# FocoosAI/focoos

Hardware: AMD Instinct MI355X
Metric: images/sec @ 640^2 (infer bs=32) (higher is better)
Workload: dtype bf16; 1 GPU; fai-detr-l-obj365 inference, bf16 MFMA, bs=32/GPU, 640x640, random-init weights (seed 0), uint8 HWC images resident in HBM, device post-process + D2H of packed detections included; global_batch=32, parallelism=replicas x1 (no data-path collective), steps_are=hipGraph replays, batches_in_flight=3, concurrent_batch_parts=1

## Files before the change

### focoos_amd/csrc/conv_pw_chain.hip

```cpp
#include "pw_common.h"

struct PwChainArgs {
  const bf16_t* x1;
  const bf16_t* x2;
  const bf16_t* res;
  const bf16_t* w1p;
  const bf16_t* w2p;
  const float* b1;
  const float* b2;
  bf16_t* y1;
  bf16_t* y2;
  int ldx1, ldx2, ldr, ldy1, ldy2;
  int M, N1, act1, act2;
  unsigned x1_bytes, x2_bytes, r_bytes;
  bf16_t* pool;
  int ldp, H, W;
};

template <int RL, typename F>
__device__ __forceinline__ void pw_dma_rows_map(__amdgpu_buffer_rsrc_t r, unsigned char* tile, int nrows, int ld, int col0, int wave, int lane, F&& pix) {
  const int ninstr = nrows * RL / 64;
  for (int i = wave; i < ninstr; i += 4) {
    const int q = i * 64 + lane;
    const int row = q / RL, pc = q % RL;
    const int lc = pw_swz<RL>(row, pc);
    const int m = pix(row);
    const unsigned off = (m >= 0) ? (unsigned)(m * ld + col0 + lc * 8) * 2u : FX_OOB;
    pw_dma16(r, tile + i * 1024, off);
  }
}

template <int K1A, int K1B, int N2, int BM, bool QUAD = false>
__global__ __launch_bounds__(256, ((N2 <= 64 && K1B == 0) ? 4 : ((N2 <= 128 && (K1B == 0 || N2 <= 64)) ? 3 : 2))) void pw_chain_kernel(const PwChainArgs p) {
  constexpr int K1 = K1A + K1B, KS1 = K1 / 16, KS1A = K1A / 16;
  constexpr int RLA = K1A / 8, RLB = (K1B > 0 ? K1B : 64) / 8;
  constexpr int TM = BM / 32;
  constexpr int XA_BYTES = BM * K1A * 2, XB_BYTES = BM * K1B * 2;
  constexpr int PF1 = KS1 < 4 ? KS1 : 4;
  constexpr bool HAS2 = N2 > 0;
  constexpr int WN2 = !HAS2 ? 1 : (N2 >= 128 ? 4 : 2), WM2 = 4 / WN2;
  constexpr int TN2 = !HAS2 ? 1 : N2 / (32 * WN2), TM2 = BM / (32 * WM2);
  constexpr int RL2 = (HAS2 ? N2 : 64) / 8;
  constexpr int PF2 = 4;
  static_assert(BM == 64, "64-pixel tiles");
  static_assert(K1A % 64 == 0 && K1B % 64 == 0 && PF1 == 4, "K segments in multiples of 64 (= whole blocks of 4 k-steps)");
  static_assert(!HAS2 || (N2 % 64 == 0 && N2 <= 256), "N2");
  extern __shared__ __attribute__((aligned(16))) unsigned char smem[];
  unsigned char* XA = smem;
  unsigned char* XB = smem + XA_BYTES;
  unsigned char* T = smem + XA_BYTES + XB_BYTES;

  const int tid = threadIdx.x, lane = tid & 63;
  const int wave = __builtin_amdgcn_readfirstlane(tid >> 6);
  const int l32 = lane & 31, half = lane >> 5;
  const int m0 = blockIdx.x * BM;
  const int NG = p.N1 >> 8;
  const int KS2 = p.N1 >> 4;

  __shared__ int s_pix[QUAD ? BM : 1];
  if constexpr (QUAD) {
    if (tid < BM) {
      const int W2 = p.W >> 1, QI = (p.H >> 1) * W2;
      const int q = blockIdx.x * (BM / 4) + (tid >> 2), sub = tid & 3;
      int m = -1;
      if (q * 4 < p.M) {
        const int b = q / QI, rem = q - b * QI;
        const int y2 = rem / W2, x2 = rem - y2 * W2;
        m = (b * p.H + 2 * y2 + (sub >> 1)) * p.W + 2 * x2 + (sub & 1);
      }
      s_pix[tid] = m;
    }
    __syncthreads();
  }
  auto pix = [&](int row) -> int {
    if constexpr (!QUAD) {
      const int m = m0 + row;
      return m < p.M ? m : -1;
    } else {
      return s_pix[row];
    }
  };
  const __amdgpu_buffer_rsrc_t x1r = __builtin_amdgcn_make_buffer_rsrc((void*)p.x1, 0, p.x1_bytes, 0x00020000);
  pw_dma_rows_map<RLA>(x1r, XA, BM, p.ldx1, 0, wave, lane, pix);
  if constexpr (K1B > 0) {
    const __amdgpu_buffer_rsrc_t x2r = __builtin_amdgcn_make_buffer_rsrc((void*)p.x2, 0, p.x2_bytes, 0x00020000);
    pw_dma_rows_map<RLB>(x2r, XB, BM, p.ldx2, 0, wave, lane, pix);
  }
  const __amdgpu_buffer_rsrc_t rr = __builtin_amdgcn_make_buffer_rsrc((void*)(p.res ? p.res : p.x1), 0, p.res ? p.r_bytes : 0u, 0x00020000);

  const int wn2 = wave % WN2, wm2 = wave / WN2;
  f32x16 acc2[TN2][TM2];
#pragma unroll
  for (int a = 0; a < TN2; ++a)
#pragma unroll
    for (int b = 0; b < TM2; ++b)
#pragma unroll
      for (int r = 0; r < 16; ++r) acc2[a][b][r] = 0.0f;

  for (int g = 0; g < NG; ++g) {
    int l32g = l32, halfg = half, tidg = tid;
    asm volatile("" : "+v"(l32g), "+v"(halfg), "+v"(tidg));
    if (p.res) pw_dma_rows_map<32>(rr, T, BM, p.ldr, g * 256, wave, lane, pix);
    bf16x8 a2[PF2][TN2];
    const bf16_t* w2 = p.w2p + (size_t)((wn2 * TN2) * KS2 + g * 16) * 512 + lane * 8;
    if constexpr (HAS2) {
#pragma unroll
      for (int i = 0; i < PF2; ++i)
#pragma unroll
        for (int a = 0; a < TN2; ++a) a2[i][a] = pw_ldg_frag(w2 + (size_t)(a * KS2 + i) * 512);
    }
#pragma unroll
    for (int a = 0; a < 2; ++a) {
      const bf16_t* w1 = p.w1p + (size_t)((g * 8 + wave * 2 + a) * KS1) * 512 + lane * 8;
      bf16x8 a1[PF1];
#pragma unroll
      for (int i = 0; i < PF1; ++i) a1[i] = pw_ldg_frag(w1 + i * 512);
      f32x16 acc[TM];
#pragma unroll
      for (int gq = 0; gq < 4; ++gq) {
        const float4 bb = *reinterpret_cast<const float4*>(p.b1 + g * 256 + wave * 64 + a * 32 + 8 * gq + 4 * halfg);
#pragma unroll
        for (int b = 0; b < TM; ++b) {
          acc[b][4 * gq] = bb.x; acc[b][4 * gq + 1] = bb.y; acc[b][4 * gq + 2] = bb.z; acc[b][4 * gq + 3] = bb.w;
        }
      }
      if (a == 0) {
        asm volatile("s_waitcnt vmcnt(0)" ::: "memory");
        __syncthreads();
      }
#define FX_PW_STEPS(XT_, KROW_, RL_, KL0_)                                                                                  \
  _Pragma("unroll") for (int i = 0; i < PF1; ++i) {                                                                         \
    bf16x8 xb[TM];                                                                                                          \
    _Pragma("unroll") for (int b = 0; b < TM; ++b) {                                                                        \
      const int row = b * 32 + l32k;                                                                                         \
      xb[b] = *reinterpret_cast<const bf16x8*>((XT_) + row * ((KROW_)*2) + (pw_swz<RL_>(row, ((KL0_) + i) * 2 + halfg) << 4)); \
    }                                                                                                                       \
    _Pragma("unroll") for (int b = 0; b < TM; ++b) acc[b] = FX_MFMA_32x32x16(a1[i], xb[b], acc[b]); \
    const int kn = ks0 + i + PF1;                                                                                           \
    a1[i] = pw_ldg_frag(w1 + (kn < KS1 ? kn : KS1 - 1) * 512);  \
  }
#pragma unroll 1
      for (int ks0 = 0; ks0 < KS1; ks0 += PF1) {
        int l32k = l32g;
        asm volatile("" : "+v"(l32k));
        if (K1B == 0 || ks0 < KS1A) {
          FX_PW_STEPS(XA, K1A, RLA, ks0)
        } else {
          FX_PW_STEPS(XB, (K1B > 0 ? K1B : 64), RLB, ks0 - KS1A)
        }
      }
#undef FX_PW_STEPS
#pragma unroll
      for (int b = 0; b < TM; ++b)
#pragma unroll
        for (int gq = 0; gq < 4; ++gq) {
          const int row = b * 32 + l32g;
          const int chunk = wave * 8 + a * 4 + gq;
          unsigned char* tp = T + row * 512 + ((chunk ^ (row & 15)) << 4) + halfg * 8;
          float v0 = acc[b][4 * gq], v1 = acc[b][4 * gq + 1], v2 = acc[b][4 * gq + 2], v3 = acc[b][4 * gq + 3];
          if (p.res) {
            const uint2 r2 = *reinterpret_cast<const uint2*>(tp);
            v0 += bf16lo_to_f32(r2.x);
            v1 += bf16hi_to_f32(r2.x);
            v2 += bf16lo_to_f32(r2.y);
            v3 += bf16hi_to_f32(r2.y);
          }
          if (p.act1 == FX_ACT_RELU) {
            v0 = fmaxf(v0, 0.0f); v1 = fmaxf(v1, 0.0f); v2 = fmaxf(v2, 0.0f); v3 = fmaxf(v3, 0.0f);
          }
          uint2 o;
          o.x = pack_bf16x2(v0, v1);
          o.y = pack_bf16x2(v2, v3);
          *reinterpret_cast<uint2*>(tp) = o;
        }
    }
    __syncthreads();
#pragma unroll
    for (int i = 0; i < BM * 32 / 256; ++i) {
      const int q = tidg + i * 256;
      const int row = q >> 5, lc = q & 31;
      const uint4 v = *reinterpret_cast<const uint4*>(T + row * 512 + ((lc ^ (row & 15)) << 4));
      const int m = pix(row);
      if (m >= 0 && p.y1) *reinterpret_cast<uint4*>(p.y1 + (size_t)m * p.ldy1 + g * 256 + lc * 8) = v;
    }
    if constexpr (QUAD) {
#pragma unroll
      for (int i = 0; i < (BM / 4) * 32 / 256; ++i) {
        const int idx = tidg + i * 256;
        const int j = idx >> 5, lc = idx & 31;
        float s8[8] = {0, 0, 0, 0, 0, 0, 0, 0};
#pragma unroll
        for (int r = 0; r < 4; ++r) {
          const int row = 4 * j + r;
          float f[8];
          unpack_bf16x8(*reinterpret_cast<const uint4*>(T + row * 512 + ((lc ^ (row & 15)) << 4)), f);
#pragma unroll
          for (int e = 0; e < 8; ++e) s8[e] += f[e];
        }
#pragma unroll
        for (int e = 0; e < 8; ++e) s8[e] *= 0.25f;
        const int q = blockIdx.x * (BM / 4) + j;
        if (q * 4 < p.M) *reinterpret_cast<uint4*>(p.pool + (size_t)q * p.ldp + g * 256 + lc * 8) = pack_bf16x8(s8);
      }
    }
    if constexpr (HAS2) {
#pragma unroll
      for (int ks = 0; ks < 16; ++ks) {
        bf16x8 tb[TM2];
#pragma unroll
        for (int b = 0; b < TM2; ++b) {
          const int row = (wm2 * TM2 + b) * 32 + l32g;
          tb[b] = *reinterpret_cast<const bf16x8*>(T + row * 512 + (((ks * 2 + halfg) ^ (row & 15)) << 4));
        }
#pragma unroll
        for (int a = 0; a < TN2; ++a)
#pragma unroll
          for (int b = 0; b < TM2; ++b) acc2[a][b] = FX_MFMA_32x32x16(a2[ks % PF2][a], tb[b], acc2[a][b]);
        if (ks + PF2 < 16) {
#pragma unroll
          for (int a = 0; a < TN2; ++a) a2[ks % PF2][a] = pw_ldg_frag(w2 + (size_t)(a * KS2 + ks + PF2) * 512);
        }
      }
    }
    __syncthreads();
  }

  if constexpr (HAS2) {
#pragma unroll
    for (int a = 0; a < TN2; ++a)
#pragma unroll
      for (int gq = 0; gq < 4; ++gq) {
        const int n = (wn2 * TN2 + a) * 32 + 8 * gq + 4 * half;
        const float4 bb = *reinterpret_cast<const float4*>(p.b2 + n);
#pragma unroll
        for (int b = 0; b < TM2; ++b) {
          const int row = (wm2 * TM2 + b) * 32 + l32;
          float v0 = acc2[a][b][4 * gq] + bb.x, v1 = acc2[a][b][4 * gq + 1] + bb.y;
          float v2 = acc2[a][b][4 * gq + 2] + bb.z, v3 = acc2[a][b][4 * gq + 3] + bb.w;
          if (p.act2 == FX_ACT_RELU) {
            v0 = fmaxf(v0, 0.0f); v1 = fmaxf(v1, 0.0f); v2 = fmaxf(v2, 0.0f); v3 = fmaxf(v3, 0.0f);
          }
          uint2 o;
          o.x = pack_bf16x2(v0, v1);
          o.y = pack_bf16x2(v2, v3);
          *reinterpret_cast<uint2*>(T + row * (N2 * 2) + (pw_swz<RL2>(row, n >> 3) << 4) + half * 8) = o;
        }
      }
    __syncthreads();
#pragma unroll
    for (int i = 0; i < BM * RL2 / 256; ++i) {
      const int q = tid + i * 256;
      const int row = q / RL2, lc = q % RL2;
      const uint4 v = *reinterpret_cast<const uint4*>(T + row * (N2 * 2) + (pw_swz<RL2>(row, lc) << 4));
      const int m = pix(row);
      if (m >= 0) *reinterpret_cast<uint4*>(p.y2 + (size_t)m * p.ldy2 + lc * 8) = v;
    }
  }
}

template <int K1A, int K1B, int N2, bool QUAD = false>
static int launch_pw_chain(const PwChainArgs& a, hipStream_t stream) {
  constexpr int BM = 64;
  constexpr int SMEM = BM * (K1A + K1B) * 2 + BM * 512;
  static bool attr_set = false;
  auto kern = pw_chain_kernel<K1A, K1B, N2, BM, QUAD>;
  if (!attr_set) {
    if (hipFuncSetAttribute(reinterpret_cast<const void*>(kern), hipFuncAttributeMaxDynamicSharedMemorySize, SMEM) != hipSuccess)
      return FX_ERR_RUNTIME;
    attr_set = true;
  }
  hipLaunchKernelGGL(kern, dim3((a.M + BM - 1) / BM), dim3(256), SMEM, stream, a);
  return fx_launch_status();
}

#define FX_PW_INSTANCES(X)                                                                             \
  X(64, 0, 0) X(64, 0, 64) X(64, 0, 128) X(64, 64, 0) X(64, 64, 64) X(64, 64, 128)                     \
  X(128, 0, 0) X(128, 0, 128) X(128, 0, 256) X(128, 256, 0) X(128, 256, 128) X(128, 256, 256)          \
  X(256, 0, 0) X(256, 0, 256) X(256, 512, 0) X(256, 512, 256)

extern "C" int fx_pw_chain_supported(int K1a, int K1b, int N1, int N2) {
  if (N1 <= 0 || N1 % 256 != 0) return 0;
#define FX_PW_CASE(KA, KB, NN2) \
  if (K1a == KA && K1b == KB && N2 == NN2) return 1;
  FX_PW_INSTANCES(FX_PW_CASE)
#undef FX_PW_CASE
  return 0;
}

#define FX_PW_POOL_INSTANCES(X) X(64, 0, 128) X(128, 0, 256)

extern "C" int fx_pw_chain_pool_supported(int K1a, int K1b, int N1, int N2) {
  if (N1 <= 0 || N1 % 256 != 0) return 0;
#define FX_PW_CASE(KA, KB, NN2) \
  if (K1a == KA && K1b == KB && N2 == NN2) return 1;
  FX_PW_POOL_INSTANCES(FX_PW_CASE)
#undef FX_PW_CASE
  return 0;
}

extern "C" int fx_pw_chain_bf16(const fx_pw_chain_desc* d, fx_stream_t stream_) {
  FX_CHECK_ARG(d && d->x1 && d->w1 && d->bias1 && d->M > 0);
  FX_CHECK_ARG(d->y1 || (d->pool && d->N2 > 0));
  FX_CHECK_ARG(d->K1b == 0 || d->x2);
  FX_CHECK_ARG((d->act1 == FX_ACT_NONE || d->act1 == FX_ACT_RELU) && (d->act2 == FX_ACT_NONE || d->act2 == FX_ACT_RELU));
  FX_CHECK_ARG(d->N2 == 0 || (d->w2 && d->bias2 && d->y2));
  if (!fx_pw_chain_supported(d->K1a, d->K1b, d->N1, d->N2)) return FX_ERR_UNSUPPORTED;
  FX_CHECK_ARG(d->ldx1 >= d->K1a && d->ldx1 % 8 == 0 && (!d->y1 || (d->ldy1 >= d->N1 && d->ldy1 % 8 == 0)));
  FX_CHECK_ARG(d->K1b == 0 || (d->ldx2 >= d->K1b && d->ldx2 % 8 == 0));
  FX_CHECK_ARG(!d->residual || (d->ldr >= d->N1 && d->ldr % 8 == 0));
  FX_CHECK_ARG(d->N2 == 0 || (d->ldy2 >= d->N2 && d->ldy2 % 8 == 0));
  FX_CHECK_ARG(((uintptr_t)d->x1 % 16) == 0 && ((uintptr_t)d->x2 % 16) == 0 && ((uintptr_t)d->residual % 16) == 0);
  FX_CHECK_ARG(((uintptr_t)d->w1 % 16) == 0 && ((uintptr_t)d->w2 % 16) == 0 && ((uintptr_t)d->y1 % 16) == 0 && ((uintptr_t)d->y2 % 16) == 0);
  FX_CHECK_ARG(((uintptr_t)d->bias1 % 16) == 0 && ((uintptr_t)d->bias2 % 16) == 0);
  const int64_t x1_bytes = ((int64_t)d->M - 1) * d->ldx1 * 2 + (int64_t)d->K1a * 2;
  const int64_t x2_bytes = d->K1b ? ((int64_t)d->M - 1) * d->ldx2 * 2 + (int64_t)d->K1b * 2 : 0;
  const int64_t r_bytes = d->residual ? ((int64_t)d->M - 1) * d->ldr * 2 + (int64_t)d->N1 * 2 : 0;
  if (x1_bytes >= 0xFFFFFFF0ll || x2_bytes >= 0xFFFFFFF0ll || r_bytes >= 0xFFFFFFF0ll) return FX_ERR_UNSUPPORTED;
  PwChainArgs a;
  a.x1 = reinterpret_cast<const bf16_t*>(d->x1);
  a.x2 = reinterpret_cast<const bf16_t*>(d->x2);
  a.res = reinterpret_cast<const bf16_t*>(d->residual);
  a.w1p = reinterpret_cast<const bf16_t*>(d->w1);
  a.w2p = reinterpret_cast<const bf16_t*>(d->w2);
  a.b1 = d->bias1;
  a.b2 = d->bias2;
  a.y1 = reinterpret_cast<bf16_t*>(d->y1);
  a.y2 = reinterpret_cast<bf16_t*>(d->y2);
  a.ldx1 = d->ldx1; a.ldx2 = d->ldx2; a.ldr = d->ldr; a.ldy1 = d->ldy1; a.ldy2 = d->ldy2;
  a.M = d->M; a.N1 = d->N1; a.act1 = d->act1; a.act2 = d->act2;
  a.x1_bytes = (unsigned)x1_bytes; a.x2_bytes = (unsigned)x2_bytes; a.r_bytes = (unsigned)r_bytes;
  a.pool = reinterpret_cast<bf16_t*>(d->pool); a.ldp = d->ldp; a.H = d->img_h; a.W = d->img_w;
  hipStream_t stream = reinterpret_cast<hipStream_t>(stream_);
  if (d->pool) {
    FX_CHECK_ARG(d->img_h > 0 && d->img_w > 0 && d->img_h % 2 == 0 && d->img_w % 2 == 0 && d->M % (d->img_h * d->img_w) == 0);
    FX_CHECK_ARG(d->ldp >= d->N1 && d->ldp % 8 == 0 && ((uintptr_t)d->pool % 16) == 0);
    if (!fx_pw_chain_pool_supported(d->K1a, d->K1b, d->N1, d->N2)) return FX_ERR_UNSUPPORTED;
#define FX_PW_CASE(KA, KB, NN2) \
  if (d->K1a == KA && d->K1b == KB && d->N2 == NN2) return launch_pw_chain<KA, KB, NN2, true>(a, stream);
    FX_PW_POOL_INSTANCES(FX_PW_CASE)
#undef FX_PW_CASE
    return FX_ERR_UNSUPPORTED;
  }
#define FX_PW_CASE(KA, KB, NN2) \
  if (d->K1a == KA && d->K1b == KB && d->N2 == NN2) return launch_pw_chain<KA, KB, NN2>(a, stream);
  FX_PW_INSTANCES(FX_PW_CASE)
#undef FX_PW_CASE
  return FX_ERR_UNSUPPORTED;
}
```

### focoos_amd/csrc/conv_pw_kplane.hip

```cpp
#include <type_traits>

#include "pw_common.h"

#ifndef FX_PWK_RES_DEPTH
#define FX_PWK_RES_DEPTH 3
#endif

int fx_tune(const char* env_name, int default_value);

struct PWKArgs {
  const bf16_t* x;
  const bf16_t* wp;
  const float* bias;
  const bf16_t* res;
  bf16_t* y;
  int N, ldx, ldy, ldr, M;
  int ntg;
  int HW;
  int64_t y_bstride;
  unsigned x_bytes, r_bytes;
  int rot;
};

template <int OFF>
__device__ __forceinline__ void pwk_ldg(bf16x8& dst, unsigned voff, const bf16_t* sbase) {
  asm volatile("global_load_dwordx4 %0, %1, %2 offset:%3" : "+v"(dst) : "v"(voff), "s"(sbase), "n"(OFF) : "memory");
}
typedef __attribute__((address_space(3))) const bf16x8 pwk_lds_frag_t;
template <int IMM>
__device__ __forceinline__ bf16x8 pwk_lds_read(int addr) {
  return *reinterpret_cast<pwk_lds_frag_t*>((size_t)(unsigned)(addr + IMM));
}
__device__ __forceinline__ float pwk_act(float v, std::integral_constant<int, FX_ACT_RELU>) { return fmaxf(v, 0.0f); }
__device__ __forceinline__ float pwk_act(float v, std::integral_constant<int, FX_ACT_SILU>) { return v * __builtin_amdgcn_rcpf(1.0f + __expf(-v)); }
__device__ __forceinline__ float pwk_act(float v, std::integral_constant<int, FX_ACT_NONE>) { return v; }

template <int K, int ACT, int RESMODE, int TM = 4, int ABL = 0>
__global__ __launch_bounds__(256, TM == 4 ? 2 : 3) void conv_pw_kplane_kernel(const PWKArgs p) {
  constexpr int TN = 2, NW = 4, BM = TM * 32, BN = 256;
  constexpr int NTHR = 256, NDW = NTHR / 64;
  constexpr int KS = K / 16;
  constexpr int PLANE = BM * 16, XBYTES = 2 * KS * PLANE;
  constexpr int PF = 4;
  static_assert(KS % PF == 0 && (KS - 1) * PLANE < 65536, "plane offsets are 16-bit immediates");
  extern __shared__ __attribute__((aligned(16))) unsigned char smem[];
  float* biasL = reinterpret_cast<float*>(smem + XBYTES);

  const int tid = threadIdx.x, lane = tid & 63;
  const int wave = __builtin_amdgcn_readfirstlane(tid >> 6);
  const int l32 = lane & 31, half = lane >> 5;
  const int m0 = fx_xcd_remap(blockIdx.x, gridDim.x) * BM;
  const int nt_first = blockIdx.y * p.ntg;
  const int NT = min(p.N / BN, nt_first + p.ntg);
  const int cnt = NT - nt_first;
  const int rot = p.rot ? (int)(blockIdx.x % (unsigned)cnt) : 0;
  auto tile_of = [&](int k) { const int t = k + rot; return nt_first + (t >= cnt ? t - cnt : t); };

  for (int i = tid; i < p.N; i += NTHR) biasL[i] = p.bias ? p.bias[i] : 0.0f;
  {
    const __amdgpu_buffer_rsrc_t xr = __builtin_amdgcn_make_buffer_rsrc((void*)p.x, 0, p.x_bytes, 0x00020000);
    constexpr int NP = K / 8;
    static_assert(BM % 64 == 0, "64-row DMA blocks");
    for (int i = wave; i < (BM / 64) * NP; i += NDW) {
      const int blk = i / NP, c = i % NP;
      const int m = m0 + blk * 64 + lane;
      const int pln = (c & 1) * KS + (c >> 1);
      if constexpr (!(ABL & 16)) pw_dma16(xr, smem + pln * PLANE + blk * 1024, m < p.M ? (unsigned)(m * p.ldx + c * 8) * 2u : FX_OOB);
    }
  }
  f32x16 acc[TN][TM];
  bf16x8 ar[PF][TN];
  const unsigned wvoff = lane * 16;
  const bf16_t* wwave = p.wp + (size_t)(wave * TN) * KS * 512;
  auto w_ptr = [&](int a, int nt, int ks) -> const bf16_t* { return wwave + ((size_t)(nt * 8 + a) * KS + ks) * 512; };
#pragma unroll
  for (int a = 0; a < TN; ++a) {
    const bf16_t* w0 = w_ptr(a, tile_of(0), 0);
    c3_static_for<PF>([&](auto ic) {
      constexpr int i = decltype(ic)::value;
      ar[i][a] = bf16x8{0, 0, 0, 0, 0, 0, 0, 0};
      pwk_ldg<i * 1024>(ar[i][a], wvoff, w0);
    });
  }
  const int lds0 = (int)(unsigned)(size_t)((__attribute__((address_space(3))) unsigned char*)smem);
  int addr[TM];
#pragma unroll
  for (int b = 0; b < TM; ++b) addr[b] = lds0 + (b * 32 + l32) * 16 + half * KS * PLANE;
  asm volatile("s_waitcnt vmcnt(0)" ::: "memory");
  __syncthreads();

  for (int kt = 0; kt < cnt; ++kt) {
    const int nt = tile_of(kt);
    const int n0 = nt * BN;
    const int ntn = kt + 1 < cnt ? tile_of(kt + 1) : nt;
#pragma unroll
    for (int a = 0; a < TN; ++a)
#pragma unroll
      for (int gq = 0; gq < 4; ++gq) {
        const float4 bb = *reinterpret_cast<const float4*>(biasL + n0 + (wave * TN + a) * 32 + 8 * gq + 4 * half);
#pragma unroll
        for (int b = 0; b < TM; ++b) {
          acc[a][b][4 * gq] = bb.x; acc[a][b][4 * gq + 1] = bb.y; acc[a][b][4 * gq + 2] = bb.z; acc[a][b][4 * gq + 3] = bb.w;
        }
      }
    bf16x8 xb[2][TM];
#pragma unroll
    for (int b = 0; b < TM; ++b) xb[0][b] = pwk_lds_read<0>(addr[b]);
#pragma unroll 1
    for (int g = 0; g < KS / PF; ++g) {
      const bool last = g == KS / PF - 1;
      const bf16_t* wnext[TN];
#pragma unroll
      for (int a = 0; a < TN; ++a) wnext[a] = w_ptr(a, last ? ntn : nt, last ? 0 : (g + 1) * PF);
      const int aoff = g * PF * PLANE;
      auto kstep = [&](auto jc) {
        constexpr int j = decltype(jc)::value;
        if constexpr (TN == 1) c3_wait<(PF - 1) * TN>(ar[j][0]); else c3_wait<(PF - 1) * TN>(ar[j][0], ar[j][1]);
#pragma unroll
        for (int a = 0; a < TN; ++a) {
#pragma unroll
          for (int b = 0; b < TM; ++b) {
            if constexpr (!(ABL & 8)) acc[a][b] = FX_MFMA_32x32x16(ar[j][a], xb[j & 1][b], acc[a][b]);
            if (a == 0) {
              if constexpr (j + 1 < PF) xb[(j + 1) & 1][b] = pwk_lds_read<(j + 1) * PLANE>(addr[b] + aoff);
              else xb[0][b] = pwk_lds_read<PF * PLANE>(addr[b] + (last ? -PF * PLANE : aoff));
            }
            if constexpr (!(ABL & 1)) {
              if (b == TM - 1) pwk_ldg<j * 1024>(ar[j][a], wvoff, wnext[a]);
            }
            __builtin_amdgcn_sched_barrier(0);
          }
        }
      };
      c3_static_for<PF>(kstep);
    }
    constexpr int RD = (FX_PWK_RES_DEPTH < TM) ? FX_PWK_RES_DEPTH : TM;
    constexpr int RS = RD + 1 > TM ? TM : RD + 1;
    uint4 rr[RS][TN * 2];
    if constexpr (ABL & 4) {
#pragma unroll
      for (int i = 0; i < RS * TN * 2; ++i) (&rr[0][0])[i] = make_uint4(0, 0, 0, 0);
    }
    auto ld_res = [&](int b, uint4* dst) {
      const int m = min(m0 + b * 32 + l32, p.M - 1);
      const bf16_t* rrow = p.res + (size_t)m * p.ldr + n0 + wave * TN * 32 + half * 8;
#pragma unroll
      for (int a = 0; a < TN; ++a)
#pragma unroll
        for (int g2 = 0; g2 < 2; ++g2) dst[a * 2 + g2] = *reinterpret_cast<const uint4*>(rrow + a * 32 + g2 * 16);
    };
    if constexpr (RESMODE != 0 && !(ABL & 4)) {
#pragma unroll
      for (int b = 0; b < RD && b < TM; ++b) ld_res(b, rr[b % RS]);
    }
#pragma unroll
    for (int b = 0; b < TM; ++b) {
      if constexpr (RESMODE != 0 && !(ABL & 4)) {
        if (b + RD < TM) ld_res(b + RD, rr[(b + RD) % RS]);
      }
      const int row = b * 32 + l32;
      const int m = m0 + row;
      size_t yo = (size_t)m * p.ldy;
      if (p.y_bstride) {
        const int bb = m / p.HW;
        yo = (size_t)bb * p.y_bstride + (size_t)(m - bb * p.HW) * p.ldy;
      }
      bf16_t* yrow = p.y + yo + n0 + wave * TN * 32 + half * 8;
      const bool live = m < p.M;
#pragma unroll
      for (int a = 0; a < TN; ++a)
#pragma unroll
        for (int g2 = 0; g2 < 2; ++g2) {
          unsigned pk[2][2], rq[2][2] = {{0u, 0u}, {0u, 0u}};
          if constexpr (RESMODE != 0) {
            const uint4 R = rr[b % RS][a * 2 + g2];
            const auto s0 = __builtin_amdgcn_permlane32_swap(R.x, R.z, false, false);
            const auto s1 = __builtin_amdgcn_permlane32_swap(R.y, R.w, false, false);
            rq[0][0] = s0[0]; rq[1][0] = s0[1];
            rq[0][1] = s1[0]; rq[1][1] = s1[1];
          }
#pragma unroll
          for (int q = 0; q < 2; ++q) {
            const int gq = 2 * g2 + q;
            float v[4];
            const float r[4] = {bf16lo_to_f32(rq[q][0]), bf16hi_to_f32(rq[q][0]), bf16lo_to_f32(rq[q][1]),
                                bf16hi_to_f32(rq[q][1])};
#pragma unroll
            for (int e = 0; e < 4; ++e) {
              v[e] = acc[a][b][4 * gq + e];
              if constexpr (RESMODE == 1) v[e] += r[e];
              v[e] = pwk_act(v[e], std::integral_constant<int, ACT>{});
              if constexpr (RESMODE == 3) v[e] = r[e] > 0.0f ? v[e] : 0.0f;
            }
            pk[q][0] = pack_bf16x2(v[0], v[1]);
            pk[q][1] = pack_bf16x2(v[2], v[3]);
          }
#pragma unroll
          for (int w = 0; w < 2; ++w) {
            const auto sw = __builtin_amdgcn_permlane32_swap(pk[0][w], pk[1][w], false, false);
            pk[0][w] = sw[0];
            pk[1][w] = sw[1];
          }
          if (live && !((ABL & 2) && p.M > 0)) *reinterpret_cast<uint4*>(yrow + a * 32 + g2 * 16) = make_uint4(pk[0][0], pk[0][1], pk[1][0], pk[1][1]);
        }
    }
  }
#pragma unroll
  for (int i = 0; i < PF; ++i) {
    if constexpr (TN == 1) c3_wait<0>(ar[i][0]); else c3_wait<0>(ar[i][0], ar[i][1]);
  }
}

template <int K, int ACT, int RESMODE, int TM = 4, int ABL = 0>
static int launch_pwk(PWKArgs& a, hipStream_t stream) {
  constexpr int BM = TM * 32, BN = 256;
  const int smem = BM * K * 2 + a.N * 4;
  if (smem > 160 * 1024) return FX_ERR_UNSUPPORTED;
  const int mt = (a.M + BM - 1) / BM, NT = a.N / BN;
  static const int target = fx_tune("FX_PWK_TARGET_WGS", 512);
  const int want = K == 256 ? target : target / 2;
  int groups = mt >= want * 3 / 4 ? 1 : (want + mt - 1) / mt;
  if (groups > NT) groups = NT;
  a.ntg = (NT + groups - 1) / groups;
  groups = (NT + a.ntg - 1) / a.ntg;
  static const int rot = fx_tune("FX_PWK_ROT", 1);
  a.rot = rot;
  auto kern = conv_pw_kplane_kernel<K, ACT, RESMODE, TM, ABL>;
  static int attr_smem = 0;
  if (smem > attr_smem) {
    if (hipFuncSetAttribute(reinterpret_cast<const void*>(kern), hipFuncAttributeMaxDynamicSharedMemorySize, smem) != hipSuccess) return FX_ERR_RUNTIME;
    attr_smem = smem;
  }
  hipLaunchKernelGGL(kern, dim3(mt, groups), dim3(256), smem, stream, a);
  return fx_launch_status();
}

bool fx_pw_kplane_supported(int C, int N, int mode) {
  if (N <= 0 || N % 256 != 0 || N > 4096) return false;
  static const int k512_res = fx_tune("FX_PWK_K512_RES", 1);
  if (C == 256) return mode == 0 || mode == 1 || mode == 3 || mode == 4 || mode == 5 || mode == 6;
  if (C == 512) return mode == 0 || mode == 1 || mode == 3 || (k512_res && (mode == 4 || mode == 5 || mode == 6));
  return false;
}

int fx_launch_pw_kplane(const ConvArgs& c, const bf16_t* w_frag, int mode, hipStream_t stream) {
  if (!fx_pw_kplane_supported(c.C, c.N, mode)) return FX_ERR_UNSUPPORTED;
  PWKArgs a{};
  a.x = c.x; a.wp = w_frag; a.bias = c.bias; a.res = c.res; a.y = reinterpret_cast<bf16_t*>(c.y);
  a.N = c.N; a.ldx = c.ldx; a.ldy = c.ldy; a.ldr = c.ldr; a.M = c.M;
  a.HW = c.Ho * c.Wo; a.y_bstride = c.y_bstride; a.x_bytes = c.x_bytes; a.r_bytes = c.r_bytes;
  if (c.C == 256) {
    switch (mode) {
      case 0: return launch_pwk<256, FX_ACT_RELU, 0>(a, stream);
      case 1: return launch_pwk<256, FX_ACT_SILU, 0>(a, stream);
      case 3: return launch_pwk<256, FX_ACT_NONE, 0>(a, stream);
      case 4: return launch_pwk<256, FX_ACT_RELU, 1>(a, stream);
      case 5: return launch_pwk<256, FX_ACT_NONE, 3>(a, stream);
      case 6: return launch_pwk<256, FX_ACT_NONE, 1>(a, stream);
    }
  } else {
    switch (mode) {
      case 0: return launch_pwk<512, FX_ACT_RELU, 0>(a, stream);
      case 1: return launch_pwk<512, FX_ACT_SILU, 0>(a, stream);
      case 3: return launch_pwk<512, FX_ACT_NONE, 0>(a, stream);
      case 4: return launch_pwk<512, FX_ACT_RELU, 1>(a, stream);
      case 5: return launch_pwk<512, FX_ACT_NONE, 3>(a, stream);
      case 6: return launch_pwk<512, FX_ACT_NONE, 1>(a, stream);
    }
  }
  return FX_ERR_UNSUPPORTED;
}
```

### focoos_amd/csrc/pw_common.h

```cpp
#pragma once
#include <type_traits>

#include "conv_common.h"

typedef __attribute__((address_space(3))) void pw_lds_void_t;

__device__ __forceinline__ void pw_dma16(__amdgpu_buffer_rsrc_t r, unsigned char* lds_base, unsigned voff) {
  __builtin_amdgcn_raw_ptr_buffer_load_lds(r, (pw_lds_void_t*)lds_base, 16, voff, 0, 0, 0);
}

template <int RL>
__device__ __forceinline__ int pw_swz(int row, int chunk) {
  if constexpr (RL >= 16) {
    return chunk ^ (row & 15);
  } else {
    constexpr int R = 16 / RL;
    return chunk ^ ((row / R) & (RL - 1));
  }
}

template <int RL>
__device__ __forceinline__ void pw_dma_rows(__amdgpu_buffer_rsrc_t r, unsigned char* tile, int nrows, int m0, int M, int ld, int col0,
                                            int wave, int lane) {
  const int ninstr = nrows * RL / 64;
  for (int i = wave; i < ninstr; i += 4) {
    const int q = i * 64 + lane;
    const int row = q / RL, pc = q % RL;
    const int lc = pw_swz<RL>(row, pc);
    const int m = m0 + row;
    const unsigned off = (m < M) ? (unsigned)(m * ld + col0 + lc * 8) * 2u : FX_OOB;
    pw_dma16(r, tile + i * 1024, off);
  }
}

__device__ __forceinline__ bf16x8 pw_ldg_frag(const bf16_t* p) { return *reinterpret_cast<const bf16x8*>(p); }


template <int N, int I = 0, typename F>
__device__ __forceinline__ void c3_static_for(F&& f) {
  if constexpr (I < N) {
    f(std::integral_constant<int, I>{});
    c3_static_for<N, I + 1>(f);
  }
}
template <int OFF = 0>
__device__ __forceinline__ void c3_ldg_async(bf16x8& dst, const bf16_t* ptr) {
  asm volatile("global_load_dwordx4 %0, %1, off offset:%2" : "+v"(dst) : "v"(ptr), "n"(OFF) : "memory");
}
template <int N>
__device__ __forceinline__ void c3_wait(bf16x8& f0) {
  asm volatile("s_waitcnt vmcnt(%1)" : "+v"(f0) : "n"(N));
}
template <int N>
__device__ __forceinline__ void c3_wait(bf16x8& f0, bf16x8& f1) {
  asm volatile("s_waitcnt vmcnt(%2)" : "+v"(f0), "+v"(f1) : "n"(N));
}
```

### focoos_amd/csrc/score_head.hip

```cpp
#include "pw_common.h"

struct ScoreHeadArgs {
  const bf16_t* mem;
  const uint8_t* valid;
  const bf16_t* w1p;
  const bf16_t* w2p;
  const float* b1;
  const float* gamma;
  const float* beta;
  const float* b2;
  bf16_t* om;
  float* scores;
  int ldm, ldo, S, M;
  float eps;
  unsigned mem_bytes;
};

template <int TN2>
__global__ __launch_bounds__(256, 2) void score_head_kernel(const ScoreHeadArgs p) {
  constexpr int BM = 64, TM = 2, KS = 16, PF = 4;
  extern __shared__ __attribute__((aligned(16))) unsigned char smem[];
  unsigned char* T = smem;
  float* red = reinterpret_cast<float*>(smem + BM * 512);

  const int tid = threadIdx.x, lane = tid & 63;
  const int wave = __builtin_amdgcn_readfirstlane(tid >> 6);
  const int l32 = lane & 31, half = lane >> 5;
  const int m0 = blockIdx.x * BM;

  const __amdgpu_buffer_rsrc_t mr = __builtin_amdgcn_make_buffer_rsrc((void*)p.mem, 0, p.mem_bytes, 0x00020000);
  for (int i = wave; i < BM * 32 / 64; i += 4) {
    const int q = i * 64 + lane;
    const int row = q >> 5, pc = q & 31;
    const int lc = pc ^ (row & 15);
    const int m = m0 + row;
    bool ok = m < p.M;
    if (ok && p.valid) ok = p.valid[m % p.S] != 0;
    pw_dma16(mr, T + i * 1024, ok ? (unsigned)(m * p.ldm + lc * 8) * 2u : FX_OOB);
  }

  f32x16 acc[2][TM];
#pragma unroll
  for (int a = 0; a < 2; ++a)
#pragma unroll
    for (int gq = 0; gq < 4; ++gq) {
      const float4 bb = *reinterpret_cast<const float4*>(p.b1 + wave * 64 + a * 32 + 8 * gq + 4 * half);
#pragma unroll
      for (int b = 0; b < TM; ++b) {
        acc[a][b][4 * gq] = bb.x; acc[a][b][4 * gq + 1] = bb.y; acc[a][b][4 * gq + 2] = bb.z; acc[a][b][4 * gq + 3] = bb.w;
      }
    }
  const bf16_t* w1 = p.w1p + (size_t)(wave * 2 * KS) * 512 + lane * 8;
  bf16x8 a1[PF][2];
#pragma unroll
  for (int i = 0; i < PF; ++i) {
    a1[i][0] = pw_ldg_frag(w1 + i * 512);
    a1[i][1] = pw_ldg_frag(w1 + (KS + i) * 512);
  }
  asm volatile("s_waitcnt vmcnt(0)" ::: "memory");
  __syncthreads();
#pragma unroll 1
  for (int ks0 = 0; ks0 < KS; ks0 += PF) {
    int l32k = l32;
    asm volatile("" : "+v"(l32k));
#pragma unroll
    for (int i = 0; i < PF; ++i) {
      bf16x8 xb[TM];
#pragma unroll
      for (int b = 0; b < TM; ++b) {
        const int row = b * 32 + l32k;
        xb[b] = *reinterpret_cast<const bf16x8*>(T + row * 512 + ((((ks0 + i) * 2 + half) ^ (row & 15)) << 4));
      }
#pragma unroll
      for (int a = 0; a < 2; ++a)
#pragma unroll
        for (int b = 0; b < TM; ++b) acc[a][b] = FX_MFMA_32x32x16(a1[i][a], xb[b], acc[a][b]);
      const int kn = ks0 + i + PF;
      const int kc = kn < KS ? kn : KS - 1;
      a1[i][0] = pw_ldg_frag(w1 + kc * 512);
      a1[i][1] = pw_ldg_frag(w1 + (KS + kc) * 512);
    }
  }
  const bf16_t* w2 = p.w2p + (size_t)(wave * TN2 * KS) * 512 + lane * 8;
  bf16x8 a2[PF][TN2];
#pragma unroll
  for (int i = 0; i < PF; ++i)
#pragma unroll
    for (int a = 0; a < TN2; ++a) a2[i][a] = pw_ldg_frag(w2 + (size_t)(a * KS + i) * 512);

  float mean[TM], rstd[TM];
  {
    float s[TM];
#pragma unroll
    for (int b = 0; b < TM; ++b) {
      float t = 0.0f;
#pragma unroll
      for (int a = 0; a < 2; ++a)
#pragma unroll
        for (int r = 0; r < 16; ++r) t += acc[a][b][r];
      t += __shfl_xor(t, 32);
      s[b] = t;
    }
    __syncthreads();
    if (half == 0) {
#pragma unroll
      for (int b = 0; b < TM; ++b) red[wave * 64 + b * 32 + l32] = s[b];
    }
    __syncthreads();
#pragma unroll
    for (int b = 0; b < TM; ++b) {
      const int r = b * 32 + l32;
      mean[b] = (red[r] + red[64 + r] + red[128 + r] + red[192 + r]) * (1.0f / 256.0f);
    }
#pragma unroll
    for (int b = 0; b < TM; ++b) {
      float t = 0.0f;
#pragma unroll
      for (int a = 0; a < 2; ++a)
#pragma unroll
        for (int r = 0; r < 16; ++r) {
          const float d = acc[a][b][r] - mean[b];
          t += d * d;
        }
      t += __shfl_xor(t, 32);
      s[b] = t;
    }
    __syncthreads();
    if (half == 0) {
#pragma unroll
      for (int b = 0; b < TM; ++b) red[wave * 64 + b * 32 + l32] = s[b];
    }
    __syncthreads();
#pragma unroll
    for (int b = 0; b < TM; ++b) {
      const int r = b * 32 + l32;
      rstd[b] = rsqrtf((red[r] + red[64 + r] + red[128 + r] + red[192 + r]) * (1.0f / 256.0f) + p.eps);
    }
  }
#pragma unroll
  for (int a = 0; a < 2; ++a)
#pragma unroll
    for (int gq = 0; gq < 4; ++gq) {
      const int n = wave * 64 + a * 32 + 8 * gq + 4 * half;
      const float4 gg = *reinterpret_cast<const float4*>(p.gamma + n);
      const float4 be = *reinterpret_cast<const float4*>(p.beta + n);
#pragma unroll
      for (int b = 0; b < TM; ++b) {
        const int row = b * 32 + l32;
        const float v0 = (acc[a][b][4 * gq] - mean[b]) * rstd[b] * gg.x + be.x;
        const float v1 = (acc[a][b][4 * gq + 1] - mean[b]) * rstd[b] * gg.y + be.y;
        const float v2 = (acc[a][b][4 * gq + 2] - mean[b]) * rstd[b] * gg.z + be.z;
        const float v3 = (acc[a][b][4 * gq + 3] - mean[b]) * rstd[b] * gg.w + be.w;
        uint2 o;
        o.x = pack_bf16x2(v0, v1);
        o.y = pack_bf16x2(v2, v3);
        *reinterpret_cast<uint2*>(T + row * 512 + (((n >> 3) ^ (row & 15)) << 4) + half * 8) = o;
      }
    }
  __syncthreads();
#pragma unroll
  for (int i = 0; i < BM * 32 / 256; ++i) {
    const int q = tid + i * 256;
    const int row = q >> 5, lc = q & 31;
    const uint4 v = *reinterpret_cast<const uint4*>(T + row * 512 + ((lc ^ (row & 15)) << 4));
    const int m = m0 + row;
    if (m < p.M) *reinterpret_cast<uint4*>(p.om + (size_t)m * p.ldo + lc * 8) = v;
  }
  f32x16 acc2[TN2][TM];
#pragma unroll
  for (int a = 0; a < TN2; ++a)
#pragma unroll
    for (int gq = 0; gq < 4; ++gq) {
      const float4 bb = *reinterpret_cast<const float4*>(p.b2 + (wave * TN2 + a) * 32 + 8 * gq + 4 * half);
#pragma unroll
      for (int b = 0; b < TM; ++b) {
        acc2[a][b][4 * gq] = bb.x; acc2[a][b][4 * gq + 1] = bb.y; acc2[a][b][4 * gq + 2] = bb.z; acc2[a][b][4 * gq + 3] = bb.w;
      }
    }
#pragma unroll 1
  for (int ks0 = 0; ks0 < KS; ks0 += PF) {
    int l32k = l32;
    asm volatile("" : "+v"(l32k));
#pragma unroll
    for (int i = 0; i < PF; ++i) {
      bf16x8 tb[TM];
#pragma unroll
      for (int b = 0; b < TM; ++b) {
        const int row = b * 32 + l32k;
        tb[b] = *reinterpret_cast<const bf16x8*>(T + row * 512 + ((((ks0 + i) * 2 + half) ^ (row & 15)) << 4));
      }
#pragma unroll
      for (int a = 0; a < TN2; ++a)
#pragma unroll
        for (int b = 0; b < TM; ++b) acc2[a][b] = FX_MFMA_32x32x16(a2[i][a], tb[b], acc2[a][b]);
      const int kn = ks0 + i + PF;
      const int kc = kn < KS ? kn : KS - 1;
#pragma unroll
      for (int a = 0; a < TN2; ++a) a2[i][a] = pw_ldg_frag(w2 + (size_t)(a * KS + kc) * 512);
    }
  }
  float mx[TM];
#pragma unroll
  for (int b = 0; b < TM; ++b) {
    float t = acc2[0][b][0];
#pragma unroll
    for (int a = 0; a < TN2; ++a)
#pragma unroll
      for (int r = 0; r < 16; ++r) t = fmaxf(t, acc2[a][b][r]);
    t = fmaxf(t, __shfl_xor(t, 32));
    mx[b] = t;
  }
  __syncthreads();
  if (half == 0) {
#pragma unroll
    for (int b = 0; b < TM; ++b) red[wave * 64 + b * 32 + l32] = mx[b];
  }
  __syncthreads();
  if (tid < BM && m0 + tid < p.M) p.scores[m0 + tid] = fmaxf(fmaxf(red[tid], red[64 + tid]), fmaxf(red[128 + tid], red[192 + tid]));
}

template <int TN2>
static int launch_score_head(const ScoreHeadArgs& a, hipStream_t stream) {
  constexpr int SMEM = 64 * 512 + 4 * 64 * 4;
  static bool attr_set = false;
  auto kern = score_head_kernel<TN2>;
  if (!attr_set) {
    if (hipFuncSetAttribute(reinterpret_cast<const void*>(kern), hipFuncAttributeMaxDynamicSharedMemorySize, SMEM) != hipSuccess)
      return FX_ERR_RUNTIME;
    attr_set = true;
  }
  hipLaunchKernelGGL(kern, dim3((a.M + 63) / 64), dim3(256), SMEM, stream, a);
  return fx_launch_status();
}

extern "C" int fx_enc_score_head_bf16(const void* memory, int ldm, const uint8_t* valid, int S, const void* w1, const float* b1,
                                      const float* gamma, const float* beta, float eps, const void* w2, const float* b2, int n2_pad,
                                      void* output_memory, int ldo, float* scores, int M, fx_stream_t stream_) {
  FX_CHECK_ARG(memory && w1 && b1 && gamma && beta && w2 && b2 && output_memory && scores && M > 0 && S > 0);
  FX_CHECK_ARG(ldm >= 256 && ldm % 8 == 0 && ldo >= 256 && ldo % 8 == 0);
  FX_CHECK_ARG(((uintptr_t)memory % 16) == 0 && ((uintptr_t)w1 % 16) == 0 && ((uintptr_t)w2 % 16) == 0 && ((uintptr_t)output_memory % 16) == 0);
  FX_CHECK_ARG(((uintptr_t)b1 % 16) == 0 && ((uintptr_t)b2 % 16) == 0 && ((uintptr_t)gamma % 16) == 0 && ((uintptr_t)beta % 16) == 0);
  if (n2_pad != 128 && n2_pad != 256 && n2_pad != 384) return FX_ERR_UNSUPPORTED;
  const int64_t mem_bytes = ((int64_t)M - 1) * ldm * 2 + 512;
  if (mem_bytes >= 0xFFFFFFF0ll) return FX_ERR_UNSUPPORTED;
  ScoreHeadArgs a;
  a.mem = reinterpret_cast<const bf16_t*>(memory);
  a.valid = valid;
  a.w1p = reinterpret_cast<const bf16_t*>(w1);
  a.w2p = reinterpret_cast<const bf16_t*>(w2);
  a.b1 = b1; a.gamma = gamma; a.beta = beta; a.b2 = b2;
  a.om = reinterpret_cast<bf16_t*>(output_memory);
  a.scores = scores;
  a.ldm = ldm; a.ldo = ldo; a.S = S; a.M = M; a.eps = eps;
  a.mem_bytes = (unsigned)mem_bytes;
  hipStream_t stream = reinterpret_cast<hipStream_t>(stream_);
  if (n2_pad == 128) return launch_score_head<1>(a, stream);
  if (n2_pad == 256) return launch_score_head<2>(a, stream);
  return launch_score_head<3>(a, stream);
}
```

Baseline: 5143 images/s.

## Software-pipeline weight loads and LDS fragment reads in pointwise chain and score head

Replaces compiler-managed weight fragment loads with inline-asm global loads that use a scalar base plus a per-lane offset, and places explicit vmcnt waits so MFMA only stalls on the fragment it needs. LDS activation reads are double-buffered one k-step ahead, and first-layer weights are prefetched across both output halves in one ring. Bias initialisation now uses scalar loads. The intent is to hide global and LDS latency behind MFMA and cut address arithmetic. In exchange the hand-counted waitcnt values must stay correct, and register pressure rises.

```diff
diff --git a/focoos_amd/csrc/conv_pw_chain.hip b/focoos_amd/csrc/conv_pw_chain.hip
--- a/focoos_amd/csrc/conv_pw_chain.hip
+++ b/focoos_amd/csrc/conv_pw_chain.hip
@@ -56,6 +56,7 @@
   const int m0 = blockIdx.x * BM;
   const int NG = p.N1 >> 8;
   const int KS2 = p.N1 >> 4;
+  const unsigned wvoff = lane * 16;
 
   __shared__ int s_pix[QUAD ? BM : 1];
   if constexpr (QUAD) {
@@ -102,54 +103,69 @@
     asm volatile("" : "+v"(l32g), "+v"(halfg), "+v"(tidg));
     if (p.res) pw_dma_rows_map<32>(rr, T, BM, p.ldr, g * 256, wave, lane, pix);
     bf16x8 a2[PF2][TN2];
-    const bf16_t* w2 = p.w2p + (size_t)((wn2 * TN2) * KS2 + g * 16) * 512 + lane * 8;
+    const bf16_t* w2g = p.w2p + (size_t)((wn2 * TN2) * KS2 + g * 16) * 512;
     if constexpr (HAS2) {
-#pragma unroll
-      for (int i = 0; i < PF2; ++i)
-#pragma unroll
-        for (int a = 0; a < TN2; ++a) a2[i][a] = pw_ldg_frag(w2 + (size_t)(a * KS2 + i) * 512);
-    }
+      c3_static_for<PF2>([&](auto ic) {
+        constexpr int i = decltype(ic)::value;
+#pragma unroll
+        for (int a = 0; a < TN2; ++a) {
+          pwk_ldg_first<i * 1024>(a2[i][a], wvoff, w2g + (size_t)(a * KS2) * 512);
+        }
+      });
+    }
+    const bf16_t* w1g = p.w1p + (size_t)((g * 8 + wave * 2) * KS1) * 512;
+    bf16x8 a1[PF1];
+    c3_static_for<PF1>([&](auto ic) {
+      constexpr int i = decltype(ic)::value;
+      pwk_ldg_first<i * 1024>(a1[i], wvoff, w1g);
+    });
+    static_assert(K1B == 0 || RLA == RLB || (RLA >= 16 && RLB >= 16), "one swizzle rule for both X tiles");
+    auto ldx = [&](bf16x8* dst, int l32k, int kn) {
+      const bool seg_a = K1B == 0 || kn < KS1A;
+      const int tile = seg_a ? 0 : XA_BYTES, rowb = seg_a ? K1A * 2 : (K1B > 0 ? K1B : 64) * 2;
+      const int c = (seg_a ? kn : kn - KS1A) * 2 + halfg;
+#pragma unroll
+      for (int b = 0; b < TM; ++b) {
+        const int row = b * 32 + l32k;
+        dst[b] = *reinterpret_cast<const bf16x8*>(smem + tile + row * rowb + (pw_swz<RLA>(row, c) << 4));
+      }
+    };
 #pragma unroll
     for (int a = 0; a < 2; ++a) {
-      const bf16_t* w1 = p.w1p + (size_t)((g * 8 + wave * 2 + a) * KS1) * 512 + lane * 8;
-      bf16x8 a1[PF1];
-#pragma unroll
-      for (int i = 0; i < PF1; ++i) a1[i] = pw_ldg_frag(w1 + i * 512);
       f32x16 acc[TM];
-#pragma unroll
-      for (int gq = 0; gq < 4; ++gq) {
-        const float4 bb = *reinterpret_cast<const float4*>(p.b1 + g * 256 + wave * 64 + a * 32 + 8 * gq + 4 * halfg);
-#pragma unroll
-        for (int b = 0; b < TM; ++b) {
-          acc[b][4 * gq] = bb.x; acc[b][4 * gq + 1] = bb.y; acc[b][4 * gq + 2] = bb.z; acc[b][4 * gq + 3] = bb.w;
-        }
-      }
+      pw_acc_from_bias<TM>(acc, p.b1 + g * 256 + wave * 64 + a * 32, halfg);
       if (a == 0) {
         asm volatile("s_waitcnt vmcnt(0)" ::: "memory");
         __syncthreads();
       }
-#define FX_PW_STEPS(XT_, KROW_, RL_, KL0_)                                                                                  \
-  _Pragma("unroll") for (int i = 0; i < PF1; ++i) {                                                                         \
-    bf16x8 xb[TM];                                                                                                          \
-    _Pragma("unroll") for (int b = 0; b < TM; ++b) {                                                                        \
-      const int row = b * 32 + l32k;                                                                                         \
-      xb[b] = *reinterpret_cast<const bf16x8*>((XT_) + row * ((KROW_)*2) + (pw_swz<RL_>(row, ((KL0_) + i) * 2 + halfg) << 4)); \
-    }                                                                                                                       \
-    _Pragma("unroll") for (int b = 0; b < TM; ++b) acc[b] = FX_MFMA_32x32x16(a1[i], xb[b], acc[b]); \
-    const int kn = ks0 + i + PF1;                                                                                           \
-    a1[i] = pw_ldg_frag(w1 + (kn < KS1 ? kn : KS1 - 1) * 512);  \
-  }
+      bf16x8 xb[2][TM];
+      ldx(xb[0], l32g, 0);
 #pragma unroll 1
       for (int ks0 = 0; ks0 < KS1; ks0 += PF1) {
         int l32k = l32g;
         asm volatile("" : "+v"(l32k));
-        if (K1B == 0 || ks0 < KS1A) {
-          FX_PW_STEPS(XA, K1A, RLA, ks0)
-        } else {
-          FX_PW_STEPS(XB, (K1B > 0 ? K1B : 64), RLB, ks0 - KS1A)
-        }
-      }
-#undef FX_PW_STEPS
+        const bool last = a == 1 && ks0 + PF1 >= KS1;
+        const bf16_t* wnext = w1g + (size_t)(a * KS1 + ks0 + (last ? 0 : PF1)) * 512;
+        const int knext = ks0 + PF1 < KS1 ? ks0 + PF1 : 0;
+        c3_static_for<PF1>([&](auto ic) {
+          constexpr int i = decltype(ic)::value;
+          ldx(xb[(i + 1) & 1], l32k, i + 1 < PF1 ? ks0 + i + 1 : knext);
+          c3_wait<PF1 - 1>(a1[i]);
+#pragma unroll
+          for (int b = 0; b < TM; ++b) acc[b] = FX_MFMA_32x32x16(a1[i], xb[i & 1][b], acc[b]);
+          pwk_ldg<i * 1024>(a1[i], wvoff, wnext);
+        });
+      }
+      if (a == 1) {
+        c3_wait<0>(a1[0], a1[1]);
+        c3_wait<0>(a1[2], a1[3]);
+        if constexpr (HAS2) {
+#pragma unroll
+          for (int i = 0; i < PF2; ++i)
+#pragma unroll
+            for (int t = 0; t < TN2; ++t) c3_landed(a2[i][t]);
+        }
+      }
 #pragma unroll
       for (int b = 0; b < TM; ++b)
 #pragma unroll
@@ -204,23 +220,31 @@
       }
     }
     if constexpr (HAS2) {
-#pragma unroll
-      for (int ks = 0; ks < 16; ++ks) {
-        bf16x8 tb[TM2];
+      bf16x8 tb[2][TM2];
+      auto ldt = [&](bf16x8* dst, int ks) {
 #pragma unroll
         for (int b = 0; b < TM2; ++b) {
           const int row = (wm2 * TM2 + b) * 32 + l32g;
-          tb[b] = *reinterpret_cast<const bf16x8*>(T + row * 512 + (((ks * 2 + halfg) ^ (row & 15)) << 4));
+          dst[b] = *reinterpret_cast<const bf16x8*>(T + row * 512 + (((ks * 2 + halfg) ^ (row & 15)) << 4));
+        }
+      };
+      ldt(tb[0], 0);
+      c3_static_for<16>([&](auto kc) {
+        constexpr int ks = decltype(kc)::value, sl = ks % PF2;
+        if constexpr (ks + 1 < 16) ldt(tb[(ks + 1) & 1], ks + 1);
+        if constexpr (ks >= PF2) {
+          constexpr int younger = (ks - 1 < 15 - PF2 ? ks - 1 : 15 - PF2) - (ks - PF2);
+          c3_wait_slot<younger * TN2, TN2>(a2[sl]);
         }
 #pragma unroll
         for (int a = 0; a < TN2; ++a)
 #pragma unroll
-          for (int b = 0; b < TM2; ++b) acc2[a][b] = FX_MFMA_32x32x16(a2[ks % PF2][a], tb[b], acc2[a][b]);
-        if (ks + PF2 < 16) {
-#pragma unroll
-          for (int a = 0; a < TN2; ++a) a2[ks % PF2][a] = pw_ldg_frag(w2 + (size_t)(a * KS2 + ks + PF2) * 512);
-        }
-      }
+          for (int b = 0; b < TM2; ++b) acc2[a][b] = FX_MFMA_32x32x16(a2[sl][a], tb[ks & 1][b], acc2[a][b]);
+        if constexpr (ks + PF2 < 16) {
+#pragma unroll
+          for (int a = 0; a < TN2; ++a) pwk_ldg<0>(a2[sl][a], wvoff, w2g + (size_t)(a * KS2 + ks + PF2) * 512);
+        }
+      });
     }
     __syncthreads();
   }
diff --git a/focoos_amd/csrc/conv_pw_kplane.hip b/focoos_amd/csrc/conv_pw_kplane.hip
--- a/focoos_amd/csrc/conv_pw_kplane.hip
+++ b/focoos_amd/csrc/conv_pw_kplane.hip
@@ -22,10 +22,6 @@
   int rot;
 };
 
-template <int OFF>
-__device__ __forceinline__ void pwk_ldg(bf16x8& dst, unsigned voff, const bf16_t* sbase) {
-  asm volatile("global_load_dwordx4 %0, %1, %2 offset:%3" : "+v"(dst) : "v"(voff), "s"(sbase), "n"(OFF) : "memory");
-}
 typedef __attribute__((address_space(3))) const bf16x8 pwk_lds_frag_t;
 template <int IMM>
 __device__ __forceinline__ bf16x8 pwk_lds_read(int addr) {
diff --git a/focoos_amd/csrc/pw_common.h b/focoos_amd/csrc/pw_common.h
--- a/focoos_amd/csrc/pw_common.h
+++ b/focoos_amd/csrc/pw_common.h
@@ -55,3 +55,40 @@
 __device__ __forceinline__ void c3_wait(bf16x8& f0, bf16x8& f1) {
   asm volatile("s_waitcnt vmcnt(%2)" : "+v"(f0), "+v"(f1) : "n"(N));
 }
+template <int N>
+__device__ __forceinline__ void c3_wait(bf16x8& f0, bf16x8& f1, bf16x8& f2) {
+  asm volatile("s_waitcnt vmcnt(%3)" : "+v"(f0), "+v"(f1), "+v"(f2) : "n"(N));
+}
+template <int N, int TN>
+__device__ __forceinline__ void c3_wait_slot(bf16x8 (&f)[TN]) {
+  static_assert(TN >= 1 && TN <= 3, "ring slots of 1 - 3 fragments");
+  if constexpr (TN == 1) c3_wait<N>(f[0]);
+  else if constexpr (TN == 2) c3_wait<N>(f[0], f[1]);
+  else c3_wait<N>(f[0], f[1], f[2]);
+}
+__device__ __forceinline__ void c3_landed(bf16x8& f0) { asm volatile("" : "+v"(f0)); }
+
+template <int OFF>
+__device__ __forceinline__ void pwk_ldg(bf16x8& dst, unsigned voff, const bf16_t* sbase) {
+  asm volatile("global_load_dwordx4 %0, %1, %2 offset:%3" : "+v"(dst) : "v"(voff), "s"(sbase), "n"(OFF) : "memory");
+}
+
+template <int OFF>
+__device__ __forceinline__ void pwk_ldg_first(bf16x8& dst, unsigned voff, const bf16_t* sbase) {
+  asm volatile("global_load_dwordx4 %0, %1, %2 offset:%3" : "=v"(dst) : "v"(voff), "s"(sbase), "n"(OFF) : "memory");
+}
+
+typedef __attribute__((address_space(4))) const float pw_sfloat_t;
+template <int TM>
+__device__ __forceinline__ void pw_acc_from_bias(f32x16 (&acc)[TM], const float* b32, int half) {
+  pw_sfloat_t* s = (pw_sfloat_t*)b32;
+#pragma unroll
+  for (int gq = 0; gq < 4; ++gq)
+#pragma unroll
+    for (int j = 0; j < 4; ++j) {
+      const float lo = s[8 * gq + j], hi = s[8 * gq + 4 + j];
+      const float v = half ? hi : lo;
+#pragma unroll
+      for (int b = 0; b < TM; ++b) acc[b][4 * gq + j] = v;
+    }
+}
diff --git a/focoos_amd/csrc/score_head.hip b/focoos_amd/csrc/score_head.hip
--- a/focoos_amd/csrc/score_head.hip
+++ b/focoos_amd/csrc/score_head.hip
@@ -50,43 +50,57 @@
         acc[a][b][4 * gq] = bb.x; acc[a][b][4 * gq + 1] = bb.y; acc[a][b][4 * gq + 2] = bb.z; acc[a][b][4 * gq + 3] = bb.w;
       }
     }
-  const bf16_t* w1 = p.w1p + (size_t)(wave * 2 * KS) * 512 + lane * 8;
+  const unsigned wvoff = lane * 16;
+  const bf16_t* w1 = p.w1p + (size_t)(wave * 2 * KS) * 512;
   bf16x8 a1[PF][2];
-#pragma unroll
-  for (int i = 0; i < PF; ++i) {
-    a1[i][0] = pw_ldg_frag(w1 + i * 512);
-    a1[i][1] = pw_ldg_frag(w1 + (KS + i) * 512);
-  }
+  c3_static_for<PF>([&](auto ic) {
+    constexpr int i = decltype(ic)::value;
+#pragma unroll
+    for (int a = 0; a < 2; ++a) {
+      pwk_ldg_first<i * 1024>(a1[i][a], wvoff, w1 + (size_t)(a * KS) * 512);
+    }
+  });
   asm volatile("s_waitcnt vmcnt(0)" ::: "memory");
   __syncthreads();
+  auto ldt = [&](bf16x8* dst, int l32k, int ks) {
+#pragma unroll
+    for (int b = 0; b < TM; ++b) {
+      const int row = b * 32 + l32k;
+      dst[b] = *reinterpret_cast<const bf16x8*>(T + row * 512 + (((ks * 2 + half) ^ (row & 15)) << 4));
+    }
+  };
+  {
+    bf16x8 xb[2][TM];
+    ldt(xb[0], l32, 0);
 #pragma unroll 1
-  for (int ks0 = 0; ks0 < KS; ks0 += PF) {
-    int l32k = l32;
-    asm volatile("" : "+v"(l32k));
-#pragma unroll
-    for (int i = 0; i < PF; ++i) {
-      bf16x8 xb[TM];
-#pragma unroll
-      for (int b = 0; b < TM; ++b) {
-        const int row = b * 32 + l32k;
-        xb[b] = *reinterpret_cast<const bf16x8*>(T + row * 512 + ((((ks0 + i) * 2 + half) ^ (row & 15)) << 4));
-      }
-#pragma unroll
-      for (int a = 0; a < 2; ++a)
-#pragma unroll
-        for (int b = 0; b < TM; ++b) acc[a][b] = FX_MFMA_32x32x16(a1[i][a], xb[b], acc[a][b]);
-      const int kn = ks0 + i + PF;
-      const int kc = kn < KS ? kn : KS - 1;
-      a1[i][0] = pw_ldg_frag(w1 + kc * 512);
-      a1[i][1] = pw_ldg_frag(w1 + (KS + kc) * 512);
-    }
-  }
-  const bf16_t* w2 = p.w2p + (size_t)(wave * TN2 * KS) * 512 + lane * 8;
+    for (int ks0 = 0; ks0 < KS; ks0 += PF) {
+      int l32k = l32;
+      asm volatile("" : "+v"(l32k));
+      const bf16_t* wnext = w1 + (size_t)(ks0 + PF < KS ? ks0 + PF : ks0) * 512;
+      c3_static_for<PF>([&](auto ic) {
+        constexpr int i = decltype(ic)::value;
+        ldt(xb[(i + 1) & 1], l32k, i + 1 < PF ? ks0 + i + 1 : (ks0 + PF < KS ? ks0 + PF : 0));
+        c3_wait<(PF - 1) * 2>(a1[i][0], a1[i][1]);
+#pragma unroll
+        for (int a = 0; a < 2; ++a)
+#pragma unroll
+          for (int b = 0; b < TM; ++b) acc[a][b] = FX_MFMA_32x32x16(a1[i][a], xb[i & 1][b], acc[a][b]);
+#pragma unroll
+        for (int a = 0; a < 2; ++a) pwk_ldg<i * 1024>(a1[i][a], wvoff, wnext + (size_t)(a * KS) * 512);
+      });
+    }
+  }
+#pragma unroll
+  for (int i = 0; i < PF; ++i) c3_wait<0>(a1[i][0], a1[i][1]);
+  const bf16_t* w2 = p.w2p + (size_t)(wave * TN2 * KS) * 512;
   bf16x8 a2[PF][TN2];
-#pragma unroll
-  for (int i = 0; i < PF; ++i)
-#pragma unroll
-    for (int a = 0; a < TN2; ++a) a2[i][a] = pw_ldg_frag(w2 + (size_t)(a * KS + i) * 512);
+  c3_static_for<PF>([&](auto ic) {
+    constexpr int i = decltype(ic)::value;
+#pragma unroll
+    for (int a = 0; a < TN2; ++a) {
+      pwk_ldg_first<i * 1024>(a2[i][a], wvoff, w2 + (size_t)(a * KS) * 512);
+    }
+  });
 
   float mean[TM], rstd[TM];
   {
@@ -177,28 +191,29 @@
         acc2[a][b][4 * gq] = bb.x; acc2[a][b][4 * gq + 1] = bb.y; acc2[a][b][4 * gq + 2] = bb.z; acc2[a][b][4 * gq + 3] = bb.w;
       }
     }
+  {
+    bf16x8 tb[2][TM];
+    ldt(tb[0], l32, 0);
 #pragma unroll 1
-  for (int ks0 = 0; ks0 < KS; ks0 += PF) {
-    int l32k = l32;
-    asm volatile("" : "+v"(l32k));
-#pragma unroll
-    for (int i = 0; i < PF; ++i) {
-      bf16x8 tb[TM];
-#pragma unroll
-      for (int b = 0; b < TM; ++b) {
-        const int row = b * 32 + l32k;
-        tb[b] = *reinterpret_cast<const bf16x8*>(T + row * 512 + ((((ks0 + i) * 2 + half) ^ (row & 15)) << 4));
-      }
-#pragma unroll
-      for (int a = 0; a < TN2; ++a)
-#pragma unroll
-        for (int b = 0; b < TM; ++b) acc2[a][b] = FX_MFMA_32x32x16(a2[i][a], tb[b], acc2[a][b]);
-      const int kn = ks0 + i + PF;
-      const int kc = kn < KS ? kn : KS - 1;
-#pragma unroll
-      for (int a = 0; a < TN2; ++a) a2[i][a] = pw_ldg_frag(w2 + (size_t)(a * KS + kc) * 512);
-    }
-  }
+    for (int ks0 = 0; ks0 < KS; ks0 += PF) {
+      int l32k = l32;
+      asm volatile("" : "+v"(l32k));
+      const bf16_t* wnext = w2 + (size_t)(ks0 + PF < KS ? ks0 + PF : ks0) * 512;
+      c3_static_for<PF>([&](auto ic) {
+        constexpr int i = decltype(ic)::value;
+        ldt(tb[(i + 1) & 1], l32k, i + 1 < PF ? ks0 + i + 1 : (ks0 + PF < KS ? ks0 + PF : 0));
+        c3_wait_slot<(PF - 1) * TN2, TN2>(a2[i]);
+#pragma unroll
+        for (int a = 0; a < TN2; ++a)
+#pragma unroll
+          for (int b = 0; b < TM; ++b) acc2[a][b] = FX_MFMA_32x32x16(a2[i][a], tb[i & 1][b], acc2[a][b]);
+#pragma unroll
+        for (int a = 0; a < TN2; ++a) pwk_ldg<i * 1024>(a2[i][a], wvoff, wnext + (size_t)(a * KS) * 512);
+      });
+    }
+  }
+#pragma unroll
+  for (int i = 0; i < PF; ++i) c3_wait_slot<0, TN2>(a2[i]);
   float mx[TM];
 #pragma unroll
   for (int b = 0; b < TM; ++b) {
```

New measurement: 5178 images/s, median of 5. No clear change (+0.7%).
